# dkogan/libdogleg

Hardware: AMD Instinct MI355X
Metric: trust-region steps/sec (fp64) at fixed (Nmeas,Nstate,nnz) (higher is better)
Workload: dtype f64

## Files before the change

include/dlg_backend.h:

```cpp
#ifndef DLG_BACKEND_H
#define DLG_BACKEND_H

#include <stddef.h>

#ifdef __cplusplus
extern "C" {
#endif

typedef struct dlg_backend dlg_backend_t;

enum
{
  DLG_OK           = 0,
  DLG_ERR_HIP      = 1,
  DLG_ERR_ARG      = 2,
  DLG_ERR_STATE    = 3,
  DLG_ERR_NOMEM    = 4,
  DLG_ERR_NODEVICE = 5,
  DLG_ERR_COMM     = 6
};

enum { DLG_DENSE = 0, DLG_SPARSE = 1, DLG_DENSE_PRODUCTS = 2 };
enum { DLG_FLAG_JTJ_PACKED = 1, DLG_FLAG_JTJ_UPPER = 2 };
enum { DLG_KIND_CAUCHY_TO_EDGE = 0, DLG_KIND_GAUSSNEWTON = 1, DLG_KIND_INTERPOLATED = 2 };
// ... 31 lines not shown
int  dlg_backend_comm_size(dlg_backend_t* b, int* nranks);
int  dlg_backend_has_rccl(dlg_backend_t* b);
int  dlg_backend_set_noop_comm(dlg_backend_t* b, int on);

int  dlg_run_steps(dlg_backend_t* b, int from, int to, int nsteps, int ncopy, const double* const* x_dev,
                   const double* const* J_dev, int first_copy, double trustregion, double lambda0,
                   double* out9, int* kind_out);

int  dlg_backend_reset(dlg_backend_t* b);
int  dlg_backend_device(dlg_backend_t* b);
int  dlg_sparse_pattern_matches(dlg_backend_t* b, const int* colptr, const int* rowidx);
int  dlg_sparse_drop_pattern(dlg_backend_t* b);

int  dlg_sparse_set_pattern(dlg_backend_t* b, const int* colptr, const int* rowidx);
int  dlg_sparse_stats(dlg_backend_t* b, long* nnz_JtJ_lower, long* nnz_L,
                      int* n_supernodes, int* n_levels, double* factor_flops);

int  dlg_sparse_region_probe(int N, int M, const int* colptr, const int* rowidx, int ncu, long* stats, int nstats);

int  dlg_sparse_schedule(dlg_backend_t* b, int* n_levels, int* persist_level0, int* persist_items);

int  dlg_sparse_leaf_rows_stats(dlg_backend_t* b, long* stats, int nstats);

int  dlg_sparse_symbolic_probe(int N, int M, const int* colptr, const int* rowidx, int row0,
                               int row1, long* stats, int nstats, int* perm_out);

int  dlg_point_set_p(dlg_backend_t* b, int slot, const double* p_host);
int  dlg_point_upload(dlg_backend_t* b, int slot, const double* x_host,
                      const double* J_host);
int  dlg_point_upload_products(dlg_backend_t* b, int slot, double norm2x,
                               const double* Jtx_host, const double* JtJ_host);
int  dlg_point_bind_device(dlg_backend_t* b, int slot, const double* x_dev,
                           const double* J_dev);
int  dlg_point_eval(dlg_backend_t* b, int slot, double* norm2_x, double* Jtx_absmax);
int  dlg_backend_set_speculation(dlg_backend_t* b, int on);
typedef void (*dlg_between_fn)(void* cookie);
int  dlg_backend_set_between(dlg_backend_t* b, dlg_between_fn fn, void* cookie);
int  dlg_backend_between_redone(dlg_backend_t* b);
int  dlg_point_eval_early(dlg_backend_t* b, int slot, const double* x_dev, const double* J_dev, int* done);
int  dlg_backend_set_defer_tail(dlg_backend_t* b, int on);
int  dlg_step_tail_pending(dlg_backend_t* b);
int  dlg_backend_ei_source(dlg_backend_t* b, int* from_solved_system, double* pivot_ratio);
int  dlg_step_tail(dlg_backend_t* b, double* expected_improvement);
int  dlg_backend_time_allreduce(dlg_backend_t* b, size_t count, int iters, double* us_each);

int  dlg_cauchy(dlg_backend_t* b, int slot, double* norm2_updateCauchy);
// ... 98 lines not shown
```

libdogleg_amd/capi.py:

```python
import ctypes as C
import os
import numpy as np

from .ctypes_defs import (Parameters2, CholmodSparse, Trace, TraceBuffer, BatchResult, JacobianReport, JacobianEntry,
                          CB_SPARSE, CB_DENSE, CB_PRODUCTS, dptr, iptr)

HERE = os.path.dirname(os.path.abspath(__file__))
LIB_PATH = os.environ.get("DLG_TEST_LIB") or os.path.join(HERE, "libdogleg_amd.so")

DLG_OK = 0
DLG_DENSE, DLG_SPARSE, DLG_DENSE_PRODUCTS = 0, 1, 2
FLAG_PACKED, FLAG_UPPER = 1, 2
KIND_CAUCHY, KIND_GN, KIND_INTERP = 0, 1, 2
VEC_P, VEC_X, VEC_JTX, VEC_CAUCHY, VEC_GN, VEC_STEP, VEC_J, VEC_X_OWN, VEC_J_OWN = range(9)

ALLREDUCE_FN = C.CFUNCTYPE(C.c_int, C.c_void_p, C.c_size_t, C.c_void_p)

BACKEND_SYMBOLS = [
    "dlg_last_error", "dlg_device_count", "dlg_backend_create", "dlg_backend_destroy",
    "dlg_backend_set_stream", "dlg_backend_get_stream", "dlg_backend_set_shard",
    "dlg_sparse_set_pattern", "dlg_sparse_stats", "dlg_sparse_schedule", "dlg_sparse_leaf_rows_stats", "dlg_point_set_p", "dlg_point_upload",
    "dlg_point_upload_products", "dlg_point_bind_device", "dlg_point_eval", "dlg_cauchy",
    "dlg_factorize", "dlg_solve_gn", "dlg_gauss_newton", "dlg_cauchy_gauss_newton", "dlg_make_step",
    "dlg_expected_improvement", "dlg_step", "dlg_take_step", "dlg_solve_with_factor",
    "dlg_point_download", "dlg_factor_download_dense", "dlg_point_device_ptr",
    "dlg_kernel_syrk_lower", "dlg_kernel_potrf_lower", "dlg_probe_mfma_f64", "dlg_probe_mfma_f64_clock", "dlg_probe_mfma_f64_waves",
    "dlg_probe_hbm_copy", "dlg_set_trace", "dlg_mem_alloc", "dlg_mem_free", "dlg_host_alloc",
    "dlg_host_free", "dlg_mem_upload",
    "dlg_mem_download", "dlg_mem_zero", "dlg_device_sync", "dlg_sparse_symbolic_probe",
    "dlg_backend_set_profiling", "dlg_backend_get_profile", "dlg_backend_get_profile_early",
    "dlg_backend_set_allreduce", "dlg_backend_set_partition", "dlg_partition_rows", "dlg_partition_stats",
    "dlg_sparse_partition_probe", "dlg_rccl_unique_id", "dlg_backend_init_rccl", "dlg_backend_set_rccl",
    "dlg_backend_comm_size", "dlg_backend_has_rccl", "dlg_backend_set_noop_comm", "dlg_solve_multi", "dlg_pseudoinverse_chunk", "dlg_backend_set_speculation", "dlg_backend_set_defer_tail", "dlg_step_tail",
    "dlg_step_tail_pending", "dlg_backend_ei_source", "dlg_backend_set_between", "dlg_backend_between_redone", "dlg_point_eval_early",
    "dlg_backend_share_rccl", "dlg_point_gather_device", "dlg_backend_reset", "dlg_backend_device",
    "dlg_sparse_pattern_matches", "dlg_sparse_drop_pattern", "dlg_sparse_region_probe", "dlg_run_steps", "dlg_backend_time_allreduce",
    "dlg_feature_leverage", "dlg_outlierness_factors", "dlg_leverage_query", "dlg_leverage_stats",
    "dlg_covariance_blocks", "dlg_marginal_variances", "dlg_covariance_stats", "dlg_covariance_plan_seconds",
    "dlg_covariance_plan_probe", "dlg_covariance_entries", "dlg_covariance_entries_stats", "dlg_covariance_entries_probe",
    "dlg_query_covariance", "dlg_query_covariance_stats", "dlg_query_covariance_plan_seconds", "dlg_query_covariance_plan_probe",
]
PROF_NAMES = ["K1_jtx", "K3K8_norm2Jv", "K4_kernel", "K4_total", "K5_factor", "K6_solve", "K7_step", "vec"]
DOGLEG_SYMBOLS = [
    "dogleg_getDefaultParameters", "dogleg_setMaxIterations",
# ... 42 lines not shown
    L.dlg_backend_get_stream.restype = V
    L.dlg_backend_set_shard.argtypes = [V, C.c_int, C.c_int, V, V]
    L.dlg_backend_set_allreduce.argtypes = [V, V, V]
    L.dlg_backend_set_speculation.argtypes = [V, C.c_int]
    L.dlg_backend_set_defer_tail.argtypes = [V, C.c_int]
    L.dlg_step_tail.argtypes = [V, C.POINTER(C.c_double)]
    L.dlg_step_tail_pending.argtypes = [V]
    L.dlg_backend_ei_source.argtypes = [V, I, D]
    L.dlg_backend_set_partition.argtypes = [V, C.c_int, C.c_int]
    L.dlg_partition_rows.argtypes = [V, I, C.POINTER(I)]
    L.dlg_partition_stats.argtypes = [V, C.POINTER(C.c_long), C.c_int]
    L.dlg_sparse_partition_probe.argtypes = [C.c_int, C.c_int, I, I, C.c_int, C.c_int, C.POINTER(C.c_long), C.c_int, C.c_char_p]
    L.dlg_rccl_unique_id.argtypes = [V]
    L.dlg_backend_init_rccl.argtypes = [V, C.c_int, C.c_int, V]
    L.dlg_backend_set_rccl.argtypes = [V, V]
    L.dlg_backend_comm_size.argtypes = [V, I]
    L.dlg_backend_has_rccl.argtypes = [V]
    L.dlg_backend_set_noop_comm.argtypes = [V, C.c_int]
    L.dlg_backend_get_profile_early.argtypes = [V, D, C.POINTER(C.c_long), C.c_int]
    L.dlg_sparse_set_pattern.argtypes = [V, I, I]
    L.dlg_sparse_stats.argtypes = [V, C.POINTER(C.c_long), C.POINTER(C.c_long), I, I, D]
    L.dlg_sparse_schedule.argtypes = [V, I, I, I]
    L.dlg_sparse_leaf_rows_stats.argtypes = [V, C.POINTER(C.c_long), C.c_int]
    L.dlg_point_set_p.argtypes = [V, C.c_int, D]
    L.dlg_point_upload.argtypes = [V, C.c_int, D, D]
    L.dlg_point_upload_products.argtypes = [V, C.c_int, C.c_double, D, D]
    L.dlg_point_bind_device.argtypes = [V, C.c_int, V, V]
    L.dlg_point_eval.argtypes = [V, C.c_int, D, D]
    L.dlg_cauchy.argtypes = [V, C.c_int, D]
    L.dlg_factorize.argtypes = [V, C.c_int, C.c_double, I]
    L.dlg_solve_gn.argtypes = [V, C.c_int, D]
    L.dlg_gauss_newton.argtypes = [V, C.c_int, D, D]
    L.dlg_cauchy_gauss_newton.argtypes = [V, C.c_int, D, D, D]
    L.dlg_make_step.argtypes = [V, C.c_int, C.c_int, C.c_int, C.c_double, D, D, D, D]
    L.dlg_step.argtypes = [V, C.c_int, C.c_int, C.c_int, C.c_double, D, D, D, D, D]
    L.dlg_take_step.argtypes = [V, C.c_int, C.c_int, C.c_double, D, D, D]
    L.dlg_solve_with_factor.argtypes = [V, C.c_int, D, D, C.c_int]
    L.dlg_solve_multi.argtypes = [V, C.c_int, D, D, C.c_int]
    L.dlg_pseudoinverse_chunk.argtypes = [V, C.c_int, C.c_int, C.c_int, D]
    L.dlg_feature_leverage.argtypes = [V, C.c_int, C.c_int, C.c_int, C.c_int, D]
    L.dlg_outlierness_factors.argtypes = [V, C.c_int, C.c_int, C.c_int, C.c_double, D]
    L.dlg_leverage_query.argtypes = [V, C.c_int, D, C.c_int, C.c_int, C.c_int, D]
    L.dlg_leverage_stats.argtypes = [V, C.c_int, C.POINTER(C.c_long), C.POINTER(C.c_long), I]
    L.dlg_covariance_blocks.argtypes = [V, C.c_int, C.c_int, I, I, I, I, D]
    L.dlg_marginal_variances.argtypes = [V, C.c_int, D]
    L.dlg_covariance_stats.argtypes = [V, C.POINTER(C.c_long), C.POINTER(C.c_long), I]
# ... 459 lines not shown
        Jp = np.ascontiguousarray(Jp, dtype=np.int32)
        Ji = np.ascontiguousarray(Ji, dtype=np.int32)
        _ck(self.L.dlg_sparse_set_pattern(self.h, iptr(Jp), iptr(Ji)), "set_pattern")

    def stats(self):
        a, b = C.c_long(), C.c_long()
        c, d = C.c_int(), C.c_int()
        e = C.c_double()
        _ck(self.L.dlg_sparse_stats(self.h, C.byref(a), C.byref(b), C.byref(c), C.byref(d), C.byref(e)),
            "stats")
        return dict(nnz_JtJ_lower=a.value, nnz_L=b.value, n_supernodes=c.value, n_levels=d.value,
                    factor_flops=e.value)

    def schedule(self):
        a, b, c = C.c_int(), C.c_int(), C.c_int()
        _ck(self.L.dlg_sparse_schedule(self.h, C.byref(a), C.byref(b), C.byref(c)), "schedule")
        return dict(n_levels=a.value, persist_level0=b.value, persist_items=c.value)

    def leaf_rows_stats(self):
        v = (C.c_long * 4)()
        _ck(self.L.dlg_sparse_leaf_rows_stats(self.h, v, 4), "leaf_rows_stats")
        return dict(lean_launches=v[0], materialized=v[1], raw=bool(v[2]), lean_levels=v[3])

    def set_p(self, slot, p):
        p = np.ascontiguousarray(p, dtype=np.float64)
        _ck(self.L.dlg_point_set_p(self.h, slot, dptr(p)), "set_p")

    def upload(self, slot, x, J):
        x = np.ascontiguousarray(x, dtype=np.float64)
        J = np.ascontiguousarray(J, dtype=np.float64)
        self._keep = [x, J]
        _ck(self.L.dlg_point_upload(self.h, slot, dptr(x), dptr(J)), "upload")

    def upload_products(self, slot, norm2x, Jtx, JtJ):
        Jtx = np.ascontiguousarray(Jtx, dtype=np.float64)
        JtJ = np.ascontiguousarray(JtJ, dtype=np.float64)
        self._keep = [Jtx, JtJ]
        _ck(self.L.dlg_point_upload_products(self.h, slot, norm2x, dptr(Jtx), dptr(JtJ)), "upload")

    def bind_device(self, slot, x_ptr, J_ptr):
        _ck(self.L.dlg_point_bind_device(self.h, slot, C.c_void_p(x_ptr), C.c_void_p(J_ptr)), "bind")

    def eval(self, slot):
        a, b = C.c_double(), C.c_double()
        _ck(self.L.dlg_point_eval(self.h, slot, C.byref(a), C.byref(b)), "eval")
        return a.value, b.value
# ... 208 lines not shown
```

libdogleg_amd/csrc/sparse_factor.hip:

```cpp
#include "sparse_internal.h"
#include "panel_factor.h"
#include "factor_tail.h"

namespace {
#ifdef DLG_FL_PROFILE
constexpr int FL_PROF_WG = 4096;
__device__ long long g_fl_prof[32*FL_PROF_WG*8];
__device__ long long g_fl_add[FL_PROF_WG*4];
#define FL_ADD_STAMP(k) do { if(HANDOFF && threadIdx.x == 0 && blockIdx.x < FL_PROF_WG) g_fl_add[blockIdx.x*4 + (k)] = wall_clock64(); } while(0)
#define FL_STAMP(k) do { if(threadIdx.x == 0 && blockIdx.x < FL_PROF_WG) g_fl_prof[((prof_lvl & 31)*FL_PROF_WG + blockIdx.x)*8 + (k)] = wall_clock64(); } while(0)
#else
#define FL_STAMP(k)
#define FL_ADD_STAMP(k)
#endif

template <int NT, bool UT_LDS, bool HANDOFF = false>
__device__ __forceinline__ void mf_add_children(double* P, double* Wt, int ntri, int nch, int ch0,
                                                MfChild rc, const MfChild* __restrict__ mf_rec,
                                                const double* uscr, const uint16_t* __restrict__ mf_dst, int tid,
                                                int* pr_flag = nullptr, int pr_epoch = 0, DlgHandoff ho = DlgHandoff{nullptr, 0, 0}, int z0 = 0)
{
  constexpr int MF_SLOTS = (NT >= 512) ? 20 : 16;
  const int lane = tid & 63;
  for(int e = z0 + tid; e < ntri; e += NT) Wt[e] = 0.0;
// ... 586 lines not shown
#pragma unroll 2
    for(int kk = 0; kk < kc; kk += 4)
    {
#pragma unroll
      for(int q = 0; q < TPW; q++)
        if(q < nmine)
          c4[q] = __builtin_amdgcn_mfma_f64_16x16x4f64(base[kk*LDB + aoff[q]], base[kk*LDB + boff[q]], c4[q], 0, 0, 0);
    }
  }
#pragma unroll
  for(int q = 0; q < TPW; q++)
    if(q < nmine)
    {
      const int j = boff[q] + jn;
#pragma unroll
      for(int r = 0; r < 4; r++)
      {
        const int i = aoff[q] + kq + 4*r;
        if(i < mb && j <= i) U[tri_col(j, mb) + i] = c4[q][r];
      }
    }
}
constexpr int GATHER_FLIGHT = 4;
template <int NT>
__global__ void __launch_bounds__(NT) k_update_gather(int unit0, const GatherUnit* __restrict__ units,
                                                       const SymSub* __restrict__ usub,
                                                       const int64_t* __restrict__ usub_u,
                                                       const int* __restrict__ relpos,
                                                       double* __restrict__ Lx,
                                                       double* __restrict__ upart,
                                                       const double* __restrict__ uscr, int nw,
                                                       int* __restrict__ info,
                                                       const int* __restrict__ fin_gate = nullptr, int fin_epoch = 0, int* fin_status = nullptr)
{
  extern __shared__ __attribute__((aligned(16))) double lds[];
  __shared__ int s_skip;
  int fin_seen = fin_epoch;
  if(fin_gate && threadIdx.x == 0) fin_seen = __hip_atomic_load(fin_gate, __ATOMIC_RELAXED, __HIP_MEMORY_SCOPE_AGENT);
  if(threadIdx.x == 0)
  {
    s_skip = *info != 0x7fffffff;
  }
  const GatherUnit U0 = units[unit0 + blockIdx.x];
  const int nc = U0.nc, nrows_t = U0.nrows_t, s0 = U0.s0, s1 = U0.s1;
  double* Lt = Lx + U0.lt;
  const int64_t part = U0.part;
  const int tid = threadIdx.x, lane = tid & 63;
  const int w = __builtin_amdgcn_readfirstlane(tid >> 6);
  const int slab = nrows_t*nc;
  for(int e = tid; e < slab*nw; e += NT) lds[e] = 0.0;
  __syncthreads();
  if(s_skip) return;
  if(w < nw)
  {
    double* acc = lds + (size_t)w*slab;
    const int nmine = (s1 - s0 - w + nw - 1)/nw;
    for(int k0 = 0; k0 < nmine; k0 += 64)
    {
      const int stl = s0 + w + (k0 + min(lane, nmine - k0 - 1))*nw;
      const SymSub R = usub[stl];
      const int64_t ru = usub_u[stl];
      const int r_rel = R.rel, r_mb = R.nrows_d - R.wd, r_m = R.m;
      const int r_ulo = (int)(uint32_t)ru, r_uhi = (int)(ru >> 32);
      const int nb = min(64, nmine - k0);
      for(int k = 0; k < nb; k += GATHER_FLIGHT)
      {
        int relv[GATHER_FLIGHT], mbv[GATHER_FLIGHT], mv[GATHER_FLIGHT], mmax = 0;
        const double* Uv[GATHER_FLIGHT];
#pragma unroll
        for(int g = 0; g < GATHER_FLIGHT; g++)
        {
          const int kg = min(k + g, nb - 1);
          relv[g] = __builtin_amdgcn_readlane(r_rel, kg);
          mbv[g] = __builtin_amdgcn_readlane(r_mb, kg);
          mv[g] = (k + g < nb) ? __builtin_amdgcn_readlane(r_m, kg) : 0;
          Uv[g] = uscr + (int64_t)(((uint64_t)(uint32_t)__builtin_amdgcn_readlane(r_uhi, kg) << 32) | (uint32_t)__builtin_amdgcn_readlane(r_ulo, kg));
          mmax = max(mmax, mv[g]);
        }
        int mv2[GATHER_FLIGHT];
#pragma unroll
        for(int g = 0; g < GATHER_FLIGHT; g++) mv2[g] = max(mv[g], 1);
        for(int i0 = 0; i0 < mmax; i0 += 64)
        {
          const int i = i0 + lane;
          const int cmax = (i < nc - 1) ? i : nc - 1;
          int ig[GATHER_FLIGHT], rg[GATHER_FLIGHT];
          double v[GATHER_FLIGHT][8];
#pragma unroll
          for(int g = 0; g < GATHER_FLIGHT; g++) { ig[g] = min(i, max(mv[g], 1) - 1); rg[g] = relpos[relv[g] + ig[g]]; }
#pragma unroll
          for(int g = 0; g < GATHER_FLIGHT; g++)
#pragma unroll
            for(int c = 0; c < 8; c++)
              if(c < nc) { const int cc = min(min(c, cmax), ig[g]); v[g][c] = Uv[g][ig[g] + cc*(mv2[g] - 1) - cc*(cc - 1)/2]; }
#pragma unroll
          for(int g = 0; g < GATHER_FLIGHT; g++)
#pragma unroll
            for(int c = 0; c < 8; c++)
              if(c < nc) { if(i < mv[g] && c <= cmax) acc[rg[g] + c*nrows_t] += v[g][c]; }
        }
      }
    }
  }
  if(fin_gate && tid == 0)
    for(int spins = 0; fin_seen != fin_epoch; spins++)
    {
      if(spins > (1 << 21)) { atomicOr(fin_status, DLG_HANDOFF_FACTOR); break; }
      __builtin_amdgcn_s_sleep(8);
      fin_seen = __hip_atomic_load(fin_gate, __ATOMIC_ACQUIRE, __HIP_MEMORY_SCOPE_AGENT);
    }
  __syncthreads();
  for(int e0 = tid; e0 < slab; e0 += 8*NT)
  {
    double old[8], tot[8];
#pragma unroll
    for(int u = 0; u < 8; u++) old[u] = (part < 0 && e0 + u*NT < slab) ? Lt[e0 + u*NT] : 0.0;
#pragma unroll
    for(int u = 0; u < 8; u++)
    {
      tot[u] = 0.0;
      if(e0 + u*NT < slab) for(int k = 0; k < nw; k++) tot[u] += lds[(size_t)k*slab + e0 + u*NT];
    }
#pragma unroll
    for(int u = 0; u < 8; u++)
      if(e0 + u*NT < slab) { if(part < 0) Lt[e0 + u*NT] = old[u] - tot[u]; else upart[part + e0 + u*NT] = tot[u]; }
  }
}

constexpr int UPD_TILES = 6;
__global__ void __launch_bounds__(TPB) k_update_mfma(int unit0, const int* __restrict__ uw_item,
                                                     const int* __restrict__ uw_s0,
                                                     const int* __restrict__ uw_s1,
                                                     const int64_t* __restrict__ uw_part,
                                                     const int* __restrict__ ui_t,
                                                     const int* __restrict__ ui_col,
                                                     const int* __restrict__ ui_nc,
                                                     const SymSub* __restrict__ usub,
                                                     const int* __restrict__ relpos,
                                                     const int* __restrict__ sn_rowptr,
                                                     const int64_t* __restrict__ sn_lx,
                                                     double* __restrict__ Lx,
                                                     double* __restrict__ upart, int nw, const int* __restrict__ info)
{
  extern __shared__ __attribute__((aligned(16))) double lds[];
  if(*info != 0x7fffffff) return;

  const int unit = unit0 + blockIdx.x;
  const int item = uw_item[unit];
  const int t = ui_t[item], col = ui_col[item], nc = ui_nc[item];
// ... 258 lines not shown
  if(!R.dst)  { DLG_CHECK(upload(R.dst, P.dst));   Y->allocs.push_back(R.dst); }
  return DLG_OK;
}
static int region_flags(dlg_backend* b, PrRegion& R)
{
  SparseSym* Y = b->sym;
  if(R.level0 >= Y->H.nlevels || R.flag) return DLG_OK;
  DLG_HIP(hipMalloc(&R.flag, sizeof(int)*((size_t)R.nwg + 1)));
  Y->allocs.push_back(R.flag);
  DLG_HIP(hipMemsetAsync(R.flag, 0, sizeof(int)*((size_t)R.nwg + 1), b->stream));
  R.epoch = 0;
  return DLG_OK;
}

int sparse_factor_setup(dlg_backend* b)
{
  SparseSym* Y = b->sym;
  const SymHost& H = Y->H;
  const RegionKnobs K = region_knobs_env(b->ncu);
  char err[256];
  if(fac_level_params(H, Y->fac, err, sizeof(err))) { dlg_set_error("%s", err); return DLG_ERR_ARG; }
  if(!Y->uw_flat && !H.uw_item.empty())
  {
    std::vector<GatherUnit> fl(H.uw_item.size());
    for(size_t u = 0; u < fl.size(); u++)
    {
      const int item = H.uw_item[u], t = H.ui_t[item];
      const int nr = H.sn_rowptr[t+1] - H.sn_rowptr[t];
      fl[u] = GatherUnit{ H.sn_lx[t] + (int64_t)H.ui_col[item]*nr, H.uw_part[u], H.uw_s0[u], H.uw_s1[u], nr, H.ui_nc[item] };
    }
    DLG_CHECK(upload(Y->uw_flat, fl)); Y->allocs.push_back(Y->uw_flat);
  }
  const bool part = H.part_nranks > 1;
  const RegionPlan top = region_plan(H, Y->fac, part ? H.cut_level + 1 : 1, H.nlevels - 1, K);
  DLG_CHECK(region_upload(b, Y->top, top));
  bool acc_any = top.acc_any;
  Y->lo.level0 = H.nlevels;
  if(part && H.cut_level >= 2 && K.lower)
  {
    const RegionPlan lo = region_plan(H, Y->fac, 1, H.cut_level, K);
    DLG_CHECK(region_upload(b, Y->lo, lo));
    acc_any = acc_any || lo.acc_any;
  }
  if(acc_any && !Y->pr_acc)
  {
    DLG_HIP(hipMalloc(&Y->pr_acc, sizeof(double)*(size_t)std::max<int64_t>(1, H.uscr_size)));
    Y->allocs.push_back(Y->pr_acc);
  }
  DLG_CHECK(region_flags(b, Y->top));
  DLG_CHECK(region_flags(b, Y->lo));
  const bool store_rows = env_int("DOGLEG_AMD_LEAF_STORE_ROWS", 0) != 0, sym_debug = getenv("DOGLEG_AMD_SYM_DEBUG") != nullptr;
  Y->leaf_lean.assign(H.nlevels, 0);
  for(int l = 0; l < H.nlevels && !store_rows; l++)
  {
    const bool own_launch = l < Y->top.level0 && !(l >= Y->lo.level0 && l <= Y->lo.level1);
    const int nu = H.uw_lvl_ptr[l+1] - H.uw_lvl_ptr[l];
    const bool rows_unread = nu == 0 || (H.upd_syrk[l] && Y->fac.upd_nw[l] > 0 && Y->fac.syrk_fused[l]);
    Y->leaf_lean[l] = (Y->fac.leaf[l] && own_launch && rows_unread) ? 1 : 0;
    if(sym_debug) fprintf(stderr, "factor level %d: lean leaf rows %d\n", l, (int)Y->leaf_lean[l]);
  }
  if(!Y->leaf_rd) { DLG_HIP(hipMalloc(&Y->leaf_rd, sizeof(double)*2*(size_t)std::max(1, H.N))); Y->allocs.push_back(Y->leaf_rd); }
  Y->leaf_rows.reset();
  const void* const big_lds[] = { (const void*)&k_factor_level<128>, (const void*)&k_factor_level<256>, (const void*)&k_factor_level<256, true>,
                                  (const void*)&k_factor_level<512>, (const void*)&k_leaf_rows_materialize<256>, (const void*)&k_update_level, (const void*)&k_update_syrk<256>,
                                  (const void*)&k_update_syrk<1024>, (const void*)&k_update_gather<TPB>, (const void*)&k_update_mfma };
  for(int i = 0; i < 10; i++) DLG_HIP(hipFuncSetAttribute(big_lds[i], hipFuncAttributeMaxDynamicSharedMemorySize, i < 5 ? FAC_LDS_BUDGET : LDS_BUDGET));
  return DLG_OK;
}

#ifdef DLG_FL_PROFILE
extern "C" void dlg_fl_profile_dump(int nlevels)
{
  std::vector<long long> h(32*FL_PROF_WG*8);
  hipDeviceSynchronize();
  hipMemcpyFromSymbol(h.data(), HIP_SYMBOL(g_fl_prof), sizeof(long long)*h.size());
  for(int l = 0; l < nlevels && l < 32; l++)
  {
    int nwg = 0, last = -1; long long t0 = 0, tend = 0; double mean[5] = {0, 0, 0, 0, 0};
    for(int g = 0; g < FL_PROF_WG; g++)
    {
      const long long* q = &h[(l*FL_PROF_WG + g)*8];
      if(q[5] == 0) continue;
      nwg++;
      if(t0 == 0 || q[0] < t0) t0 = q[0];
      if(q[5] > tend) { tend = q[5]; last = g; }
      for(int k = 0; k < 5; k++) mean[k] += (double)(q[k+1] - q[k]);
    }
    if(nwg == 0) continue;
// ... 10 lines not shown
      }
      fprintf(stderr, "   wg %3d (w %3lld rows %4lld nch %lld u_lds %lld lvl %lld rep %lld): start %6lld flag up %6lld panel in %6lld added %6lld factored %6lld tail %6lld flag+stored %6lld\n",
              g, q[6] & 4095, (q[6] >> 12) & 4095, (q[6] >> 24) & 4095, (q[6] >> 36) & 1, (q[6] >> 56) & 63, (q[6] >> 52) & 15, q[0] - t0, q[7] - t0, q[1] - t0, q[2] - t0, q[3] - t0, q[4] - t0, q[5] - t0);
    }
    const long long* q = &h[(l*FL_PROF_WG + last)*8];
    fprintf(stderr, "level %2d: %3d wg, span %7lld | last wg %3d (w %3lld rows %4lld slice %4lld nch %2lld u_lds %lld has_u %lld): start +%6lld load %6lld add %6lld factor %6lld tail %6lld store %6lld | mean: load %6.0f add %6.0f factor %6.0f tail %6.0f store %6.0f\n",
            l, nwg, tend - t0, last, q[6] & 4095, (q[6] >> 12) & 4095, (q[6] >> 40) & 4095, (q[6] >> 24) & 4095, (q[6] >> 36) & 1, (q[6] >> 37) & 1,
            q[0] - t0, q[1] - q[0], q[2] - q[1], q[3] - q[2], q[4] - q[3], q[5] - q[4],
            mean[0]/nwg, mean[1]/nwg, mean[2]/nwg, mean[3]/nwg, mean[4]/nwg);
  }
  std::vector<long long> z(h.size(), 0);
  hipMemcpyToSymbol(HIP_SYMBOL(g_fl_prof), z.data(), sizeof(long long)*z.size());
}
#endif
int sparse_factor_levels(dlg_backend* b, int part)
{
  SparseSym* Y = b->sym;
  const SymHost& H = Y->H;
  hipStream_t st = b->stream;
  const bool split = Y->top.level0 > 0 && H.nlevels >= 2 && H.part_nranks <= 1 && H.fw_lvl_ptr[1] > H.fw_lvl_ptr[0];
  if(part == 2 && !split) return DLG_OK;
  if(part != 2)
  {
  if(H.part_nranks > 1 && H.cut_level < 0) DLG_CHECK(sparse_partition_reduce(b));
  if(Y->top.level0 == 0 || H.nlevels < 2) DLG_CHECK(sparse_fin_side_gate(b));
  }
  for(int l = 0; l < H.nlevels; l++)
  {
    const bool launched_before = part == 2 && l == 0;

    const int n = H.fw_lvl_ptr[l+1] - H.fw_lvl_ptr[l];
    const bool gate_here = (l == Y->top.level0 && Y->top.flag) || (l == Y->lo.level0 && Y->lo.flag);
    if(l > 0 && n < 256 && !gate_here) dlg_fork_point(b);
    if(l == Y->lo.level0 && Y->lo.flag)
    {
      PrRegion& R = Y->lo;
      ++R.epoch;
      if(l > 0 && n < 256) dlg_fork_gate(b, R.flag + R.nwg, R.epoch);
      {
        DlgRegionTurn turn(b);
        launch_region(b, R, l);
      }
      l = R.level1;
      if(H.part_nranks > 1 && l == H.cut_level) { DLG_LAUNCH_CHECK(); DLG_CHECK(sparse_partition_reduce(b)); }
      continue;
    }
// ... 14 lines not shown
      launch_factor_level(Y->fac.nt[l], Y->fac.leaf[l], n, Y->fac.lds[l], st, Y, Y->fw_item + H.fw_lvl_ptr[l], Y->mf_rec, Y->mf_dst,
                          fmode, (int*)nullptr, 0, DlgHandoff{nullptr, 0, 0}, (int64_t)0, lean ? Y->leaf_rd + (size_t)rd_slot*H.N : (double*)nullptr);
      if(lean) Y->leaf_rows.factored_lean(Y->Lx);
      else if(Y->fac.leaf[l]) Y->leaf_rows.factored_full(Y->Lx);
    }
    if(part == 1 && split && l == 0) { Y->fac_pending = true; DLG_LAUNCH_CHECK(); return DLG_OK; }
    const int nu = H.uw_lvl_ptr[l+1] - H.uw_lvl_ptr[l];
    const bool gather_next = nu > 0 && H.upd_syrk[l] && Y->fac.upd_nw[l] > 0;
    const int fin_ep = (l == 0 && gather_next) ? Y->fin_side_owed : 0;
    if(fin_ep) Y->fin_side_owed = 0;
    if(l == 0) DLG_CHECK(sparse_fin_side_gate(b));
    if(gather_next)
    {
      const int ns = H.xl_ptr[l+1] - H.xl_ptr[l];
      if(Y->fac.syrk_fused[l] || ns == 0) {  }
      else if(Y->fac.syrk_nt[l] == 256)
        hipLaunchKernelGGL(HIP_KERNEL_NAME(k_update_syrk<256>), dim3(ns), dim3(256), Y->fac.syrk_lds[l], st,
                           Y->xl_sn + H.xl_ptr[l], Y->sn_c0, Y->sn_rowptr, Y->sn_lx, Y->u_off, Y->Lx, Y->uscr,
                           Y->fac.syrk_kc[l]);
      else
        hipLaunchKernelGGL(HIP_KERNEL_NAME(k_update_syrk<1024>), dim3(ns), dim3(1024), Y->fac.syrk_lds[l], st,
                           Y->xl_sn + H.xl_ptr[l], Y->sn_c0, Y->sn_rowptr, Y->sn_lx, Y->u_off, Y->Lx, Y->uscr,
                           Y->fac.syrk_kc[l]);
      hipLaunchKernelGGL(HIP_KERNEL_NAME(k_update_gather<TPB>), dim3(nu), dim3(TPB), Y->fac.upd_lds[l], st, H.uw_lvl_ptr[l],
                         Y->uw_flat, Y->usub, Y->usub_u, Y->relpos, Y->Lx, Y->upart, Y->uscr,
                         Y->fac.upd_nw[l], Y->d_info,
                         fin_ep ? (const int*)(Y->fin_flag + 1) : (const int*)nullptr, fin_ep,
                         reinterpret_cast<int*>(b->d_scal + (dlg_backend::NSCAL - 2)));
    }
    else if(nu > 0 && Y->fac.upd_coop[l] == 2)
      hipLaunchKernelGGL(k_update_mfma, dim3(nu), dim3(TPB), Y->fac.upd_lds[l], st, H.uw_lvl_ptr[l],
                         Y->uw_item, Y->uw_s0, Y->uw_s1, Y->uw_part, Y->ui_t, Y->ui_col, Y->ui_nc,
                         Y->usub, Y->relpos, Y->sn_rowptr, Y->sn_lx, Y->Lx, Y->upart, Y->fac.upd_nw[l], (const int*)Y->d_info);
    else if(nu > 0 && Y->fac.upd_coop[l])
      hipLaunchKernelGGL(k_update_coop, dim3(nu), dim3(TPB), 0, st, H.uw_lvl_ptr[l],
                         Y->uw_item, Y->uw_s0, Y->uw_s1, Y->uw_part, Y->ui_t, Y->ui_col, Y->ui_nc,
                         Y->usub, Y->relpos, Y->sn_rowptr, Y->sn_lx, Y->Lx, Y->upart, (const int*)Y->d_info);
    else if(nu > 0)
      hipLaunchKernelGGL(k_update_level, dim3(nu), dim3(TPB), Y->fac.upd_lds[l], st, H.uw_lvl_ptr[l],
                         Y->uw_item, Y->uw_s0, Y->uw_s1, Y->uw_part, Y->ui_t, Y->ui_col, Y->ui_nc,
                         Y->usub, Y->relpos, Y->sn_rowptr, Y->sn_lx, Y->Lx, Y->upart, Y->fac.upd_nw[l], (const int*)Y->d_info);
    const int nfz = H.uf_lvl_ptr[l+1] - H.uf_lvl_ptr[l];
    if(nfz > 0)
      hipLaunchKernelGGL(k_update_fin, dim3(nfz, Y->fac.fin_ny[l]), dim3(TPB), 0, st, H.uf_lvl_ptr[l], Y->uf_item, Y->uf_n,
                         Y->uf_off, Y->ui_t, Y->ui_col, Y->ui_nc, Y->sn_rowptr, Y->sn_lx, Y->Lx,
                         Y->upart, (const int*)Y->d_info);
    if(H.part_nranks > 1 && l == H.cut_level) { DLG_LAUNCH_CHECK(); DLG_CHECK(sparse_partition_reduce(b)); }
  }
  if(!H.ms_sn.empty())
    hipLaunchKernelGGL(k_copy_top, dim3((unsigned)H.ms_sn.size()), dim3(TPB), 0, st, Y->ms_sn, Y->sn_c0,
                       Y->sn_rowptr, Y->sn_lx, Y->sn_top, Y->Lx, Y->top_scr, (const int*)Y->d_info);
  DLG_LAUNCH_CHECK();
  return DLG_OK;
}

int sparse_leaf_rows_materialize(dlg_backend* b)
{
  SparseSym* Y = b->sym;
  if(!Y || !Y->Lx || !Y->leaf_rows.raw(Y->Lx)) return DLG_OK;
  const SymHost& H = Y->H;
  const int slot = Y->leaf_rows.slot(Y->Lx);
  for(int l = 0; l < H.nlevels; l++)
  {
    const int n = H.fw_lvl_ptr[l+1] - H.fw_lvl_ptr[l];
    if(!Y->leaf_lean[l] || n == 0) continue;
    hipLaunchKernelGGL(HIP_KERNEL_NAME(k_leaf_rows_materialize<256>), dim3(n), dim3(256), Y->fac.lds[l], b->stream,
                       Y->fw_item + H.fw_lvl_ptr[l], Y->Lx, Y->leaf_rd + (size_t)slot*H.N, (const int*)Y->d_info);
  }
  DLG_LAUNCH_CHECK();
  Y->leaf_rows.materialize(Y->Lx);
  return DLG_OK;
}
extern "C" int dlg_sparse_leaf_rows_stats(dlg_backend_t* b, long* stats, int nstats)
{
  if(!b || !b->sym || !stats) { dlg_set_error("no symbolic analysis yet"); return DLG_ERR_STATE; }
  const SparseSym* Y = b->sym;
  long lean = 0;
  for(char c : Y->leaf_lean) lean += c;
  const long v[] = { Y->leaf_rows.lean_launches, Y->leaf_rows.materialized, Y->leaf_rows.raw(Y->Lx) ? 1L : 0L, lean };
  for(int i = 0; i < nstats && i < 4; i++) stats[i] = v[i];
  return DLG_OK;
}

extern "C" int dlg_sparse_region_probe(int N, int M, const int* colptr, const int* rowidx, int ncu, long* stats, int nstats)
{
  SymHost H;
  char err[512];
  if(sym_analyze(H, N, M, colptr, rowidx, 0, M, err, sizeof(err))) { dlg_set_error("symbolic analysis: %s", err); return DLG_ERR_ARG; }
  const RegionKnobs K = region_knobs_env(ncu);
  FacLevels L;
  if(fac_level_params(H, L, err, sizeof(err))) { dlg_set_error("%s", err); return DLG_ERR_ARG; }
  const RegionPlan R = region_plan(H, L, 1, H.nlevels - 1, K);
  long checked[2];
  if(region_check(H, R, checked, err, sizeof(err))) { dlg_set_error("%s", err); return DLG_ERR_STATE; }
  const long v[] = { (long)R.level0, (long)(H.fw_lvl_ptr[H.nlevels] - H.fw_lvl_ptr[std::min(R.level0, H.nlevels)]),
                     (long)R.nwg, (long)R.lds, checked[0], checked[1], (long)region_plan_hash(R), (long)fac_levels_hash(L) };
  for(int i = 0; i < nstats && i < 8; i++) stats[i] = v[i];
  return DLG_OK;
}
```

libdogleg_amd/csrc/sparse_internal.h:

```cpp
#pragma once
#include "dlg_internal.h"
#include "sparse_symbolic.h"
#include "sparse_region.h"
#include "leaf_rows_state.h"

namespace {
constexpr int JFL_SEG = 16;
constexpr int NV_CHUNK = 2048;

constexpr int TPB = 256;
constexpr int LDS_BUDGET = SYM_LDS_BUDGET;
constexpr int FAC_LDS_BUDGET = SYM_FAC_LDS_BUDGET;

__device__ __forceinline__ double wave_sum(double v)
{
#pragma unroll
  for(int o = 32; o > 0; o >>= 1) v += __shfl_down(v, o, 64);
  return v;
}

template <int NT, int U, class LoadF, class StoreF>
__device__ __forceinline__ void batched_copy(int total, int tid, LoadF ld, StoreF st)
{
  for(int base = 0; base < total; base += U*NT)
  {
    double v[U];
#pragma unroll
    for(int u = 0; u < U; u++) { const int idx = base + u*NT + tid; v[u] = (idx < total) ? ld(idx) : 0.0; }
#pragma unroll
    for(int u = 0; u < U; u++) { const int idx = base + u*NT + tid; if(idx < total) st(idx, v[u]); }
  }
}

template <class T> int upload(T*& dev, const std::vector<T>& h)
{
  dev = nullptr;
  const size_t bytes = sizeof(T)*(h.size() ? h.size() : 1);
  DLG_HIP(hipMalloc(&dev, bytes));
  if(!h.empty()) DLG_HIP(hipMemcpy(dev, h.data(), sizeof(T)*h.size(), hipMemcpyHostToDevice));
  return DLG_OK;
}

}

struct GatherUnit { int64_t lt, part; int s0, s1, nrows_t, nc; };
struct SolveItem { int c0, w, nrows, rowoff; int64_t lx; int bd0, nbd; int pflag, rsv; };

struct PrRegion
{
  int level0 = 1 << 30, level1 = -1, lds = 0, stage = 0, nwg = 0;
  FwItem* item = nullptr; MfChild* rec = nullptr; uint16_t* dst = nullptr;
  int* flag = nullptr; int epoch = 0;
};

struct SparseSym
{
  SymHost H;
  uint64_t pat_key = 0;
  int *sn_c0 = nullptr, *sn_rowptr = nullptr, *sn_rows = nullptr, *sn_scr = nullptr, *lvl_sn = nullptr;
  int64_t *sn_lx = nullptr, *diagpos = nullptr;
  int *ui_t = nullptr, *ui_col = nullptr, *ui_nc = nullptr, *ui_ptr = nullptr;
  SymSub* usub = nullptr; int* relpos = nullptr;
  int *uw_item = nullptr, *uw_s0 = nullptr, *uw_s1 = nullptr, *uf_item = nullptr, *uf_n = nullptr;
  int64_t *uw_part = nullptr, *uf_off = nullptr;
  GatherUnit* uw_flat = nullptr;
  double* upart = nullptr; double* uscr = nullptr; int64_t *u_off = nullptr, *usub_u = nullptr;
  SolveItem* slv_item = nullptr; FwItem* fw_item = nullptr; MfChild* mf_rec = nullptr; uint16_t* mf_dst = nullptr;
  SymOutBlock* oblk = nullptr; SymContrib* contrib = nullptr;
  SymTask *jtx_task = nullptr;
  int *jtx_fin_ptr = nullptr, *jtx_fin_blk = nullptr;
  int *jtx_fin_short = nullptr, *jtx_fin_long = nullptr; int n_fin_short = 0, n_fin_long = 0;
  AsmRho* asm_rho = nullptr; AsmPair* asm_pair = nullptr; AsmSlot* asm_slot = nullptr;
  AsmBatch* asm_batch = nullptr; AsmTask* asm_ctask = nullptr; AsmFin* asm_cfin = nullptr;
  bool asm_pent_ok = false;
  uint32_t* asm_pent = nullptr;
  AsmShape* asm_shape = nullptr; AsmKG* asm_kg = nullptr; AsmMTask* asm_mtask = nullptr; int* asm_tdest = nullptr;
  int *jf_ptr = nullptr, *jf_ent = nullptr, *jf_var0 = nullptr, *jf_w = nullptr, *jf_short = nullptr, *jf_long = nullptr;
  double* jf_lpart = nullptr; int* jf_lcnt = nullptr;
  const double* fin_pending_rhs = nullptr; const double* spec_aug_rhs = nullptr; bool info_clean = false;
  double* fin_pending_Lx = nullptr;
  bool spare_dirty = false, spare_zeroed = false; hipStream_t spare_stream = nullptr;
  double* jtp = nullptr;
  AsmFin2* asm_fin2 = nullptr; int64_t* asm_fin2_list = nullptr; AsmRun* asm_run = nullptr; int* asm_pdest = nullptr;
  int *rl_ptr = nullptr, *rl_pos = nullptr, *perm = nullptr, *col_sn = nullptr;
  int *fw_sn = nullptr, *fw_r0 = nullptr, *fw_r1 = nullptr, *ms_sn = nullptr; int64_t* sn_top = nullptr;
  int *sn_bd_ptr = nullptr, *sn_bd_col = nullptr;
  double* top_scr = nullptr;
  const double* aug_rhs = nullptr;
// ... 52 lines not shown
```

Before: 1882.

## Fold multi-chunk gather partial sums in last-arriving workgroup, split columns across waves

The update-gather kernel now splits columns across waves, so each wave accumulates its own columns in LDS instead of each wave holding a full private slab that is later summed. For multi-chunk items, every chunk writes its partial to global memory and bumps an arrival counter. The last workgroup to arrive sums all partials and writes the result into L, so the separate k_update_fin launch for those levels is skipped. This removes a kernel launch and per-wave LDS reduction, at the cost of atomic counters, fences and a serialized fold in one workgroup per item. It also adds a stats query.

Result: no change. 1888 (median of 2 runs) (+0.3%).

```diff
diff --git a/include/dlg_backend.h b/include/dlg_backend.h
--- a/include/dlg_backend.h
+++ b/include/dlg_backend.h
@@ -77,6 +77,8 @@
 
 int  dlg_sparse_leaf_rows_stats(dlg_backend_t* b, long* stats, int nstats);
 
+int  dlg_sparse_update_gather_stats(dlg_backend_t* b, long* stats, int nstats);
+
 int  dlg_sparse_symbolic_probe(int N, int M, const int* colptr, const int* rowidx, int row0,
                                int row1, long* stats, int nstats, int* perm_out);
 
diff --git a/libdogleg_amd/capi.py b/libdogleg_amd/capi.py
--- a/libdogleg_amd/capi.py
+++ b/libdogleg_amd/capi.py
@@ -19,7 +19,7 @@
 BACKEND_SYMBOLS = [
     "dlg_last_error", "dlg_device_count", "dlg_backend_create", "dlg_backend_destroy",
     "dlg_backend_set_stream", "dlg_backend_get_stream", "dlg_backend_set_shard",
-    "dlg_sparse_set_pattern", "dlg_sparse_stats", "dlg_sparse_schedule", "dlg_sparse_leaf_rows_stats", "dlg_point_set_p", "dlg_point_upload",
+    "dlg_sparse_set_pattern", "dlg_sparse_stats", "dlg_sparse_schedule", "dlg_sparse_leaf_rows_stats", "dlg_sparse_update_gather_stats", "dlg_point_set_p", "dlg_point_upload",
     "dlg_point_upload_products", "dlg_point_bind_device", "dlg_point_eval", "dlg_cauchy",
     "dlg_factorize", "dlg_solve_gn", "dlg_gauss_newton", "dlg_cauchy_gauss_newton", "dlg_make_step",
     "dlg_expected_improvement", "dlg_step", "dlg_take_step", "dlg_solve_with_factor",
@@ -108,6 +108,7 @@
     L.dlg_sparse_stats.argtypes = [V, C.POINTER(C.c_long), C.POINTER(C.c_long), I, I, D]
     L.dlg_sparse_schedule.argtypes = [V, I, I, I]
     L.dlg_sparse_leaf_rows_stats.argtypes = [V, C.POINTER(C.c_long), C.c_int]
+    L.dlg_sparse_update_gather_stats.argtypes = [V, C.POINTER(C.c_long), C.c_int]
     L.dlg_point_set_p.argtypes = [V, C.c_int, D]
     L.dlg_point_upload.argtypes = [V, C.c_int, D, D]
     L.dlg_point_upload_products.argtypes = [V, C.c_int, C.c_double, D, D]
@@ -613,6 +614,11 @@
         _ck(self.L.dlg_sparse_leaf_rows_stats(self.h, v, 4), "leaf_rows_stats")
         return dict(lean_launches=v[0], materialized=v[1], raw=bool(v[2]), lean_levels=v[3])
 
+    def update_gather_stats(self):
+        v = (C.c_long * 3)()
+        _ck(self.L.dlg_sparse_update_gather_stats(self.h, v, 3), "update_gather_stats")
+        return dict(units=v[0], multi_chunk_items=v[1], folded_sums=v[2])
+
     def set_p(self, slot, p):
         p = np.ascontiguousarray(p, dtype=np.float64)
         _ck(self.L.dlg_point_set_p(self.h, slot, dptr(p)), "set_p")
diff --git a/libdogleg_amd/csrc/sparse_factor.hip b/libdogleg_amd/csrc/sparse_factor.hip
--- a/libdogleg_amd/csrc/sparse_factor.hip
+++ b/libdogleg_amd/csrc/sparse_factor.hip
@@ -632,19 +632,23 @@
     }
 }
 constexpr int GATHER_FLIGHT = 4;
+constexpr int GATHER_NT = 128;
+constexpr int GATHER_WG_PER_CU = 8;
+constexpr int GATHER_FOLD = 2;
 template <int NT>
 __global__ void __launch_bounds__(NT) k_update_gather(int unit0, const GatherUnit* __restrict__ units,
                                                        const SymSub* __restrict__ usub,
                                                        const int64_t* __restrict__ usub_u,
                                                        const int* __restrict__ relpos,
                                                        double* __restrict__ Lx,
-                                                       double* __restrict__ upart,
-                                                       const double* __restrict__ uscr, int nw,
+                                                       double* upart, int* __restrict__ arrive,
+                                                       const double* __restrict__ uscr,
                                                        int* __restrict__ info,
                                                        const int* __restrict__ fin_gate = nullptr, int fin_epoch = 0, int* fin_status = nullptr)
 {
+  constexpr int NW = NT/64, CPW = 8/NW;
   extern __shared__ __attribute__((aligned(16))) double lds[];
-  __shared__ int s_skip;
+  __shared__ int s_skip, s_last;
   int fin_seen = fin_epoch;
   if(fin_gate && threadIdx.x == 0) fin_seen = __hip_atomic_load(fin_gate, __ATOMIC_RELAXED, __HIP_MEMORY_SCOPE_AGENT);
   if(threadIdx.x == 0)
@@ -658,31 +662,40 @@
   const int tid = threadIdx.x, lane = tid & 63;
   const int w = __builtin_amdgcn_readfirstlane(tid >> 6);
   const int slab = nrows_t*nc;
-  for(int e = tid; e < slab*nw; e += NT) lds[e] = 0.0;
+  const int ncw = (nc > w) ? (nc - w + NW - 1)/NW : 0;
+  const int mine = ncw*nrows_t;
+  auto place = [&](int e) { int j = 0;
+#pragma unroll
+                            for(int q = 1; q < CPW; q++) j += (e >= q*nrows_t) ? 1 : 0;
+                            return e + (w + j*(NW - 1))*nrows_t; };
+  for(int e = lane; e < mine; e += 64) lds[place(e)] = 0.0;
   __syncthreads();
-  if(s_skip) return;
-  if(w < nw)
-  {
-    double* acc = lds + (size_t)w*slab;
-    const int nmine = (s1 - s0 - w + nw - 1)/nw;
-    for(int k0 = 0; k0 < nmine; k0 += 64)
-    {
-      const int stl = s0 + w + (k0 + min(lane, nmine - k0 - 1))*nw;
+  if(s_skip)
+  {
+    if(part >= 0 && tid == 0 && atomicAdd(arrive + U0.cnt, 1) == U0.nch - 1)
+      __hip_atomic_store(arrive + U0.cnt, 0, __ATOMIC_RELAXED, __HIP_MEMORY_SCOPE_AGENT);
+    return;
+  }
+  if(ncw > 0)
+  {
+    const int nsub = s1 - s0;
+    for(int k0 = 0; k0 < nsub; k0 += 64)
+    {
+      const int stl = s0 + k0 + min(lane, nsub - k0 - 1);
       const SymSub R = usub[stl];
       const int64_t ru = usub_u[stl];
-      const int r_rel = R.rel, r_mb = R.nrows_d - R.wd, r_m = R.m;
+      const int r_rel = R.rel, r_m = R.m;
       const int r_ulo = (int)(uint32_t)ru, r_uhi = (int)(ru >> 32);
-      const int nb = min(64, nmine - k0);
+      const int nb = min(64, nsub - k0);
       for(int k = 0; k < nb; k += GATHER_FLIGHT)
       {
-        int relv[GATHER_FLIGHT], mbv[GATHER_FLIGHT], mv[GATHER_FLIGHT], mmax = 0;
+        int relv[GATHER_FLIGHT], mv[GATHER_FLIGHT], mmax = 0;
         const double* Uv[GATHER_FLIGHT];
 #pragma unroll
         for(int g = 0; g < GATHER_FLIGHT; g++)
         {
           const int kg = min(k + g, nb - 1);
           relv[g] = __builtin_amdgcn_readlane(r_rel, kg);
-          mbv[g] = __builtin_amdgcn_readlane(r_mb, kg);
           mv[g] = (k + g < nb) ? __builtin_amdgcn_readlane(r_m, kg) : 0;
           Uv[g] = uscr + (int64_t)(((uint64_t)(uint32_t)__builtin_amdgcn_readlane(r_uhi, kg) << 32) | (uint32_t)__builtin_amdgcn_readlane(r_ulo, kg));
           mmax = max(mmax, mv[g]);
@@ -693,24 +706,37 @@
         for(int i0 = 0; i0 < mmax; i0 += 64)
         {
           const int i = i0 + lane;
-          const int cmax = (i < nc - 1) ? i : nc - 1;
           int ig[GATHER_FLIGHT], rg[GATHER_FLIGHT];
-          double v[GATHER_FLIGHT][8];
-#pragma unroll
-          for(int g = 0; g < GATHER_FLIGHT; g++) { ig[g] = min(i, max(mv[g], 1) - 1); rg[g] = relpos[relv[g] + ig[g]]; }
+          double v[GATHER_FLIGHT][CPW];
+#pragma unroll
+          for(int g = 0; g < GATHER_FLIGHT; g++) { ig[g] = min(i, mv2[g] - 1); rg[g] = relpos[relv[g] + ig[g]]; }
 #pragma unroll
           for(int g = 0; g < GATHER_FLIGHT; g++)
 #pragma unroll
-            for(int c = 0; c < 8; c++)
-              if(c < nc) { const int cc = min(min(c, cmax), ig[g]); v[g][c] = Uv[g][ig[g] + cc*(mv2[g] - 1) - cc*(cc - 1)/2]; }
+            for(int j = 0; j < CPW; j++)
+              if(j < ncw) { const int cc = min(w + j*NW, ig[g]); v[g][j] = Uv[g][ig[g] + cc*(mv2[g] - 1) - cc*(cc - 1)/2]; }
 #pragma unroll
           for(int g = 0; g < GATHER_FLIGHT; g++)
 #pragma unroll
-            for(int c = 0; c < 8; c++)
-              if(c < nc) { if(i < mv[g] && c <= cmax) acc[rg[g] + c*nrows_t] += v[g][c]; }
+            for(int j = 0; j < CPW; j++)
+              if(j < ncw) { const int c = w + j*NW; if(i < mv[g] && c <= i) lds[rg[g] + c*nrows_t] += v[g][j]; }
         }
       }
     }
+  }
+  typedef __attribute__((address_space(1))) double* gdp_t;
+  if(part >= 0)
+  {
+    for(int e = lane; e < mine; e += 64)
+    {
+      const int a = place(e);
+      __hip_atomic_store((gdp_t)(upart + part + a), lds[a], __ATOMIC_RELAXED, __HIP_MEMORY_SCOPE_AGENT);
+    }
+    asm volatile("s_waitcnt vmcnt(0)" ::: "memory");
+    __syncthreads();
+    if(tid == 0) s_last = (atomicAdd(arrive + U0.cnt, 1) == U0.nch - 1);
+    __syncthreads();
+    if(!s_last) return;
   }
   if(fin_gate && tid == 0)
     for(int spins = 0; fin_seen != fin_epoch; spins++)
@@ -720,21 +746,50 @@
       fin_seen = __hip_atomic_load(fin_gate, __ATOMIC_ACQUIRE, __HIP_MEMORY_SCOPE_AGENT);
     }
   __syncthreads();
-  for(int e0 = tid; e0 < slab; e0 += 8*NT)
-  {
-    double old[8], tot[8];
-#pragma unroll
-    for(int u = 0; u < 8; u++) old[u] = (part < 0 && e0 + u*NT < slab) ? Lt[e0 + u*NT] : 0.0;
-#pragma unroll
-    for(int u = 0; u < 8; u++)
-    {
-      tot[u] = 0.0;
-      if(e0 + u*NT < slab) for(int k = 0; k < nw; k++) tot[u] += lds[(size_t)k*slab + e0 + u*NT];
-    }
-#pragma unroll
-    for(int u = 0; u < 8; u++)
-      if(e0 + u*NT < slab) { if(part < 0) Lt[e0 + u*NT] = old[u] - tot[u]; else upart[part + e0 + u*NT] = tot[u]; }
-  }
+  if(part < 0)
+  {
+    for(int e0 = lane; e0 < mine; e0 += 8*64)
+    {
+      int a[8]; double old[8];
+#pragma unroll
+      for(int u = 0; u < 8; u++) { a[u] = place(min(e0 + u*64, mine - 1)); old[u] = Lt[a[u]]; }
+#pragma unroll
+      for(int u = 0; u < 8; u++)
+        if(e0 + u*64 < mine) Lt[a[u]] = old[u] - lds[a[u]];
+    }
+    return;
+  }
+  __builtin_amdgcn_fence(__ATOMIC_ACQUIRE, "agent");
+  const double* P0 = upart + U0.part0;
+  const int nch = U0.nch;
+  for(int e0 = tid; e0 < slab; e0 += GATHER_FOLD*NT)
+  {
+    int e[GATHER_FOLD]; double t[GATHER_FOLD], oldv[GATHER_FOLD];
+#pragma unroll
+    for(int q = 0; q < GATHER_FOLD; q++) { e[q] = min(e0 + q*NT, slab - 1); t[q] = 0.0; oldv[q] = Lt[e[q]]; }
+    for(int k0 = 0; k0 < nch; k0 += 8)
+    {
+      double pv[8][GATHER_FOLD];
+#pragma unroll
+      for(int u = 0; u < 8; u++)
+      {
+        const double* q0 = P0 + (size_t)min(k0 + u, nch - 1)*slab;
+#pragma unroll
+        for(int q = 0; q < GATHER_FOLD; q++) pv[u][q] = __hip_atomic_load((gdp_t)(q0 + e[q]), __ATOMIC_RELAXED, __HIP_MEMORY_SCOPE_AGENT);
+      }
+#pragma unroll
+      for(int u = 0; u < 8; u++)
+        if(k0 + u < nch)
+        {
+#pragma unroll
+          for(int q = 0; q < GATHER_FOLD; q++) t[q] += pv[u][q];
+        }
+    }
+#pragma unroll
+    for(int q = 0; q < GATHER_FOLD; q++)
+      if(e0 + q*NT < slab) Lt[e[q]] = oldv[q] - t[q];
+  }
+  if(tid == 0) __hip_atomic_store(arrive + U0.cnt, 0, __ATOMIC_RELAXED, __HIP_MEMORY_SCOPE_AGENT);
 }
 
 constexpr int UPD_TILES = 6;
@@ -1039,13 +1094,22 @@
   if(fac_level_params(H, Y->fac, err, sizeof(err))) { dlg_set_error("%s", err); return DLG_ERR_ARG; }
   if(!Y->uw_flat && !H.uw_item.empty())
   {
-    std::vector<GatherUnit> fl(H.uw_item.size());
-    for(size_t u = 0; u < fl.size(); u++)
-    {
-      const int item = H.uw_item[u], t = H.ui_t[item];
-      const int nr = H.sn_rowptr[t+1] - H.sn_rowptr[t];
-      fl[u] = GatherUnit{ H.sn_lx[t] + (int64_t)H.ui_col[item]*nr, H.uw_part[u], H.uw_s0[u], H.uw_s1[u], nr, H.ui_nc[item] };
-    }
+    std::vector<GatherUnit> fl;
+    fl.reserve(H.uw_item.size());
+    std::vector<int> fin_of(H.ui_t.size(), -1);
+    for(size_t f = 0; f < H.uf_item.size(); f++) fin_of[H.uf_item[f]] = (int)f;
+    for(int l = 0; l < H.nlevels; l++)
+      for(int chunks = 1; chunks >= 0; chunks--)
+        for(int u = H.uw_lvl_ptr[l]; u < H.uw_lvl_ptr[l+1]; u++)
+        {
+          if((H.uw_part[u] >= 0) != (chunks == 1)) continue;
+          const int item = H.uw_item[u], t = H.ui_t[item], f = chunks ? fin_of[item] : -1;
+          const int nr = H.sn_rowptr[t+1] - H.sn_rowptr[t];
+          fl.push_back(GatherUnit{ H.sn_lx[t] + (int64_t)H.ui_col[item]*nr, H.uw_part[u], f >= 0 ? H.uf_off[f] : -1, H.uw_s0[u], H.uw_s1[u],
+                                   nr, H.ui_nc[item], f, f >= 0 ? H.uf_n[f] : 0 });
+        }
+    const std::vector<int> zeros(H.uf_item.size(), 0);
+    DLG_CHECK(upload(Y->uw_arrive, zeros)); Y->allocs.push_back(Y->uw_arrive);
     DLG_CHECK(upload(Y->uw_flat, fl)); Y->allocs.push_back(Y->uw_flat);
   }
   const bool part = H.part_nranks > 1;
@@ -1080,7 +1144,7 @@
   Y->leaf_rows.reset();
   const void* const big_lds[] = { (const void*)&k_factor_level<128>, (const void*)&k_factor_level<256>, (const void*)&k_factor_level<256, true>,
                                   (const void*)&k_factor_level<512>, (const void*)&k_leaf_rows_materialize<256>, (const void*)&k_update_level, (const void*)&k_update_syrk<256>,
-                                  (const void*)&k_update_syrk<1024>, (const void*)&k_update_gather<TPB>, (const void*)&k_update_mfma };
+                                  (const void*)&k_update_syrk<1024>, (const void*)&k_update_gather<GATHER_NT>, (const void*)&k_update_mfma };
   for(int i = 0; i < 10; i++) DLG_HIP(hipFuncSetAttribute(big_lds[i], hipFuncAttributeMaxDynamicSharedMemorySize, i < 5 ? FAC_LDS_BUDGET : LDS_BUDGET));
   return DLG_OK;
 }
@@ -1137,6 +1201,7 @@
   if(part == 2 && !split) return DLG_OK;
   if(part != 2)
   {
+  Y->gather_stats[0] = Y->gather_stats[1] = Y->gather_stats[2] = 0;
   if(H.part_nranks > 1 && H.cut_level < 0) DLG_CHECK(sparse_partition_reduce(b));
   if(Y->top.level0 == 0 || H.nlevels < 2) DLG_CHECK(sparse_fin_side_gate(b));
   }
@@ -1197,11 +1262,13 @@
         hipLaunchKernelGGL(HIP_KERNEL_NAME(k_update_syrk<1024>), dim3(ns), dim3(1024), Y->fac.syrk_lds[l], st,
                            Y->xl_sn + H.xl_ptr[l], Y->sn_c0, Y->sn_rowptr, Y->sn_lx, Y->u_off, Y->Lx, Y->uscr,
                            Y->fac.syrk_kc[l]);
-      hipLaunchKernelGGL(HIP_KERNEL_NAME(k_update_gather<TPB>), dim3(nu), dim3(TPB), Y->fac.upd_lds[l], st, H.uw_lvl_ptr[l],
-                         Y->uw_flat, Y->usub, Y->usub_u, Y->relpos, Y->Lx, Y->upart, Y->uscr,
-                         Y->fac.upd_nw[l], Y->d_info,
+      const int gather_lds = std::max(Y->fac.upd_lds[l]/Y->fac.upd_nw[l], 163840/GATHER_WG_PER_CU);
+      hipLaunchKernelGGL(HIP_KERNEL_NAME(k_update_gather<GATHER_NT>), dim3(nu), dim3(GATHER_NT), gather_lds, st,
+                         H.uw_lvl_ptr[l], Y->uw_flat, Y->usub, Y->usub_u, Y->relpos, Y->Lx, Y->upart, Y->uw_arrive, Y->uscr, Y->d_info,
                          fin_ep ? (const int*)(Y->fin_flag + 1) : (const int*)nullptr, fin_ep,
                          reinterpret_cast<int*>(b->d_scal + (dlg_backend::NSCAL - 2)));
+      const long nf = H.uf_lvl_ptr[l+1] - H.uf_lvl_ptr[l];
+      Y->gather_stats[0] += nu; Y->gather_stats[1] += nf; Y->gather_stats[2] += nf;
     }
     else if(nu > 0 && Y->fac.upd_coop[l] == 2)
       hipLaunchKernelGGL(k_update_mfma, dim3(nu), dim3(TPB), Y->fac.upd_lds[l], st, H.uw_lvl_ptr[l],
@@ -1216,7 +1283,7 @@
                          Y->uw_item, Y->uw_s0, Y->uw_s1, Y->uw_part, Y->ui_t, Y->ui_col, Y->ui_nc,
                          Y->usub, Y->relpos, Y->sn_rowptr, Y->sn_lx, Y->Lx, Y->upart, Y->fac.upd_nw[l], (const int*)Y->d_info);
     const int nfz = H.uf_lvl_ptr[l+1] - H.uf_lvl_ptr[l];
-    if(nfz > 0)
+    if(nfz > 0 && !gather_next)
       hipLaunchKernelGGL(k_update_fin, dim3(nfz, Y->fac.fin_ny[l]), dim3(TPB), 0, st, H.uf_lvl_ptr[l], Y->uf_item, Y->uf_n,
                          Y->uf_off, Y->ui_t, Y->ui_col, Y->ui_nc, Y->sn_rowptr, Y->sn_lx, Y->Lx,
                          Y->upart, (const int*)Y->d_info);
@@ -1254,6 +1321,13 @@
   for(char c : Y->leaf_lean) lean += c;
   const long v[] = { Y->leaf_rows.lean_launches, Y->leaf_rows.materialized, Y->leaf_rows.raw(Y->Lx) ? 1L : 0L, lean };
   for(int i = 0; i < nstats && i < 4; i++) stats[i] = v[i];
+  return DLG_OK;
+}
+
+extern "C" int dlg_sparse_update_gather_stats(dlg_backend_t* b, long* stats, int nstats)
+{
+  if(!b || !b->sym || !stats) { dlg_set_error("no symbolic analysis yet"); return DLG_ERR_STATE; }
+  for(int i = 0; i < nstats && i < 3; i++) stats[i] = b->sym->gather_stats[i];
   return DLG_OK;
 }
 
diff --git a/libdogleg_amd/csrc/sparse_internal.h b/libdogleg_amd/csrc/sparse_internal.h
--- a/libdogleg_amd/csrc/sparse_internal.h
+++ b/libdogleg_amd/csrc/sparse_internal.h
@@ -43,7 +43,7 @@
 
 }
 
-struct GatherUnit { int64_t lt, part; int s0, s1, nrows_t, nc; };
+struct GatherUnit { int64_t lt, part, part0; int s0, s1, nrows_t, nc, cnt, nch; };
 struct SolveItem { int c0, w, nrows, rowoff; int64_t lx; int bd0, nbd; int pflag, rsv; };
 
 struct PrRegion
@@ -64,6 +64,8 @@
   int *uw_item = nullptr, *uw_s0 = nullptr, *uw_s1 = nullptr, *uf_item = nullptr, *uf_n = nullptr;
   int64_t *uw_part = nullptr, *uf_off = nullptr;
   GatherUnit* uw_flat = nullptr;
+  int* uw_arrive = nullptr;
+  long gather_stats[3] = {0, 0, 0};
   double* upart = nullptr; double* uscr = nullptr; int64_t *u_off = nullptr, *usub_u = nullptr;
   SolveItem* slv_item = nullptr; FwItem* fw_item = nullptr; MfChild* mf_rec = nullptr; uint16_t* mf_dst = nullptr;
   SymOutBlock* oblk = nullptr; SymContrib* contrib = nullptr;
```
